# zssjh/stereo-semantic-vo

Hardware: AMD Instinct MI355X
Metric: stereo frames/sec on KITTI 00 (full Tracking::Track chain) (higher is better)
Workload: dtype u8; 1 GPU; BASELINE configs[2]: synth-kitti00 sequence of 4541 distinct 1241x376 stereo pairs, full Tracking::Track loop per frame (ORB on L and R, sparse stereo, matching passes 1+2, PnP-RANSAC, pose-only LM, map-point lifecycle); ONE sequence per GPU in strict frame order (replicas across GPUs); parallelism=one GPU, resident_pairs_per_gpu=4541, resident_input_bytes_per_gpu=4370984960, frames_tracked=4541, tracker_capacity_flag=0, pnp_samples_through_sequential_fallback=0

## Files before the change

### stereo-semantic-vo_amd/csrc/svo_epnp_ord_asm.h

```cpp
#define EO_JACOBI_ASM_12 \
  "v_mov_b64 v[150:151], %[x0]\n\t" \
  "v_mov_b64 v[152:153], %[x1]\n\t" \
  "v_mov_b64 v[154:155], %[x2]\n\t" \
  "v_mov_b64 v[180:181], 1.0\n\t" \
  "v_mov_b32 v254, 1\n\t" \
  "ds_read_b32 v158, %[tper] offset:0\n\t" \
  "ds_read_b32 v159, %[tper] offset:48\n\t" \
  "ds_read_b32 v176, %[tper] offset:96\n\t" \
  "ds_read_b32 v177, %[tper] offset:144\n\t" \
  "ds_read_b32 v178, %[tper] offset:192\n\t" \
  "ds_read_b32 v179, %[tper] offset:240\n\t" \
  "ds_read_b32 v246, %[tper] offset:288\n\t" \
  "ds_read_b32 v247, %[tper] offset:336\n\t" \
  "ds_read_b32 v248, %[tper] offset:384\n\t" \
  "ds_read_b32 v249, %[tper] offset:432\n\t" \
  "ds_read_b32 v250, %[tper] offset:480\n\t" \
  "ds_read_b32 v251, %[tper] offset:528\n\t" \
  "v_and_b32 v228, 15, %[lane]\n\t" \
  "v_sub_u32 v230, v228, %[base]\n\t" \
  "v_cmp_ne_u32 s[60:61], 0, %[act]\n\t" \
  "s_waitcnt lgkmcnt(0)\n\t" \
  "v_and_b32 v253, 15, v158\n\t" \
  "v_cmp_ne_u32 vcc, v253, v230\n\t" \
  "s_and_b64 s[62:63], vcc, s[60:61]\n\t" \
// ... 3659 lines not shown
  "v_and_b32 v246, 0x80, v234\n\t" \
  "v_cmp_ne_u32 vcc, 0, v246\n\t" \
  "s_and_b64 s[68:69], vcc, s[60:61]\n\t" \
  "s_cbranch_scc0 L_open_%=\n\t" \
  "v_bfe_u32 v246, v234, 8, 2\n\t" \
  "v_add_u32 v246, v246, v240\n\t" \
  "v_lshrrev_b32 v247, v246, %[chg]\n\t" \
  "v_and_b32 v247, 1, v247\n\t" \
  "v_cmp_ne_u32 vcc, 0, v247\n\t" \
  "s_and_b64 s[70:71], vcc, s[68:69]\n\t" \
  "v_mov_b32 v247, s70\n\t" \
  "v_and_b32 v247, v247, %[pm]\n\t" \
  "v_cmp_eq_u32 vcc, 0, v247\n\t" \
  "v_cmp_le_u32 s[70:71], 24, v246\n\t" \
  "s_or_b64 vcc, vcc, s[70:71]\n\t" \
  "s_and_b64 vcc, vcc, s[68:69]\n\t" \
  "s_andn2_b64 s[60:61], s[60:61], vcc\n\t" \
  "s_and_b64 s[70:71], s[70:71], s[68:69]\n\t" \
  "v_cndmask_b32_e64 v246, 0, 1, s[70:71]\n\t" \
  "v_or_b32 %[flag], %[flag], v246\n\t" \
  "s_and_b64 s[62:63], s[62:63], s[60:61]\n\t" \
  "L_open_%=:\n\t" \
  "v_mov_b32 v234, v235\n\t" \
  "v_mov_b32 v240, v241\n\t" \
  "v_mov_b32 v241, v239\n\t" \
  "s_cmp_lg_u64 s[60:61], 0\n\t" \
  "s_cbranch_scc1 L_loop_%=\n\t" \
  "L_done_%=:\n\t" \
  "s_waitcnt lgkmcnt(0)\n\t" \
  "v_mov_b64 %[x0], v[150:151]\n\t" \
  "v_mov_b64 %[x1], v[152:153]\n\t" \
  "v_mov_b64 %[x2], v[154:155]\n\t"

#define EO_JACOBI_ASM_CLOBBERS "v140", "v141", "v142", "v143", "v144", "v145", "v146", "v147", "v148", "v149", "v150", "v151", "v152", "v153", "v154", "v155", "v156", "v157", "v158", "v159", "v160", "v161", "v162", "v163", "v164", "v165", "v166", "v167", "v168", "v169", "v170", "v171", "v172", "v173", "v174", "v175", "v176", "v177", "v178", "v179", "v180", "v181", "v182", "v183", "v184", "v185", "v186", "v187", "v188", "v189", "v190", "v191", "v192", "v193", "v194", "v195", "v196", "v197", "v198", "v199", "v200", "v201", "v202", "v203", "v204", "v205", "v206", "v207", "v208", "v209", "v210", "v211", "v212", "v213", "v214", "v215", "v216", "v217", "v218", "v219", "v220", "v221", "v222", "v223", "v224", "v225", "v226", "v227", "v228", "v229", "v230", "v231", "v232", "v233", "v234", "v235", "v236", "v237", "v238", "v239", "v240", "v241", "v242", "v243", "v244", "v245", "v246", "v247", "v248", "v249", "v250", "v251", "v252", "v253", "v254", "v255", "s60", "s61", "s62", "s63", "s64", "s65", "s66", "s67", "s68", "s69", "s70", "s71", "vcc", "scc", "memory"
```

### stereo-semantic-vo_amd/csrc/svo_epnp_ord_dev.h

```cpp
#pragma once
#ifndef HIP_INCLUDE_HIP_HIP_RUNTIME_H
#include <hip/hip_runtime.h>
#endif
#include <stdint.h>

#include "svo_epnp_exact_dev.h"

namespace epnp_ord {

#define EO_FN __device__ __forceinline__
typedef double d2 __attribute__((ext_vector_type(2)));

#include "svo_epnp_ord_tab.h"
#include "svo_epnp_ord_asm.h"

#define EO_SYNC()                                         \
  do {                                                    \
    __builtin_amdgcn_fence(__ATOMIC_ACQ_REL, "wavefront"); \
    __builtin_amdgcn_wave_barrier();                      \
  } while (0)

struct Lds {
  alignas(16) double jr[16 * 16];
  alignas(16) double xch[16][4][4];
  unsigned tab[EO_TAB_TOTAL];
  double pws[16], us[10], alphas[20], cws[12], ccinv[9];
  double M[120];
  double ut4[4][12];
  double L[60], rho[6];
  double sw[3][6];
  double bx[3][6];
  double ccs[3][12], pcs[3][16], abt[3][9], Rc[3][9], rep[3][8];
  alignas(16) double gn[3][6][6];
  double out[3][16];
  int srow[3][6];
  int urow[4];
  double xw[16];
  int flag;
  int sweeps;
  int why;
  long long stamp[8];
#ifdef EO_PROFILE
  long long prof[8];
#endif
};

EO_FN double xdiv(double a, double b) { return a / b; }
EO_FN double xsqrt(double x) { return sqrt(x); }

EO_FN double ndiv(double a, double b) {
  double r = __builtin_amdgcn_rcp(b);
  double e = __builtin_fma(-b, r, 1.0);
  r = __builtin_fma(r, e, r);
  e = __builtin_fma(-b, r, 1.0);
  r = __builtin_fma(r, e, r);
  const double q = a * r;
  const double rem = __builtin_fma(-b, q, a);
  return __builtin_fma(rem, r, q);
}
EO_FN double nsqrt(double x) {
  const double y = __builtin_amdgcn_rsq(x);
  double g = x * y, h = 0.5 * y;
  const double r = __builtin_fma(-h, g, 0.5);
  g = __builtin_fma(g, r, g);
  h = __builtin_fma(h, r, h);
  double d = __builtin_fma(-g, g, x);
  g = __builtin_fma(d, h, g);
  d = __builtin_fma(-g, g, x);
  g = __builtin_fma(d, h, g);
  return g;
}
EO_FN bool w_in_range(double w) { return w >= 7.888609052210118e-31 && w <= 1.2676506002282294e30; }

EO_FN double gsum(double term, double acc) { return __builtin_amdgcn_mfma_f64_4x4x4f64(1.0, term, acc, 0, 0, 0); }
template <int M>
EO_FN double colsum(double t0, double t1, double t2, int g) {
// ... 104 lines not shown
        "v_mul_f64 %[s2], %[n2], %[n2]\n\t"
        "v_mfma_f64_4x4x4_4b_f64 %[a], %[one], %[s0], 0\n\t"
        "s_nop 3\n\t"
        "v_mfma_f64_4x4x4_4b_f64 %[a], %[one], %[s1], %[a]\n\t"
        "s_nop 3\n\t"
        "v_mfma_f64_4x4x4_4b_f64 %[a], %[one], %[s2], %[a]\n\t"
        "s_nop 5"
        : [a] "=&v"(a), [s0] "=&v"(s0), [s1] "=&v"(s1), [s2] "=&v"(s2)
        : [n0] "v"(n0), [n1] "v"(n1), [n2] "v"(n2), [one] "v"(one));
  } else if (M == 6) {
    asm volatile(
        "v_mul_f64 %[s0], %[n0], %[n0]\n\t"
        "v_mul_f64 %[s1], %[n1], %[n1]\n\t"
        "v_mul_f64 %[s1], %[s1], %[mk]\n\t"
        "v_mfma_f64_4x4x4_4b_f64 %[a], %[one], %[s0], 0\n\t"
        "s_nop 3\n\t"
        "v_mfma_f64_4x4x4_4b_f64 %[a], %[one], %[s1], %[a]\n\t"
        "s_nop 5"
        : [a] "=&v"(a), [s0] "=&v"(s0), [s1] "=&v"(s1)
        : [n0] "v"(n0), [n1] "v"(n1), [mk] "v"(mk), [one] "v"(one));
  } else {
    asm volatile(
        "v_mul_f64 %[s0], %[n0], %[n0]\n\t"
        "v_mul_f64 %[s0], %[s0], %[mk]\n\t"
        "s_nop 1\n\t"
        "v_mfma_f64_4x4x4_4b_f64 %[a], %[one], %[s0], 0\n\t"
        "s_nop 5"
        : [a] "=&v"(a), [s0] "=&v"(s0)
        : [n0] "v"(n0), [mk] "v"(mk), [one] "v"(one));
  }
  return a;
}

template <int M>
EO_FN unsigned long long jacobi_rows(Lds& S, int n, int base, int lane) {
  const int r = lane & 15, g = lane >> 4, q = r - base;
  const double mk = M == 6 ? (g < 2 ? 1.0 : 0.0) : (M == 3 ? (g < 3 ? 1.0 : 0.0) : 1.0);
  const double eps = 2.220446049250313e-16 * 10;
  double x0 = S.jr[r * 16 + g], x1 = S.jr[r * 16 + 4 + g], x2 = S.jr[r * 16 + 8 + g];
  double* const mine = S.xch[r][g];
  { d2 lo; lo.x = x0; lo.y = x1; *reinterpret_cast<d2*>(mine) = lo; mine[2] = x2; }
  const int tb = n == 12 ? EO_TAB12_OFF : (n == 5 ? EO_TAB5_OFF : (n == 4 ? EO_TAB4_OFF : EO_TAB3_OFF));
  const int steps = n == 12 ? EO_TAB12_STEPS : (n == 5 ? EO_TAB5_STEPS : (n == 4 ? EO_TAB4_STEPS : EO_TAB3_STEPS));
  const int pro = n == 12 ? EO_TAB12_PROLOGUE : (n == 5 ? EO_TAB5_PROLOGUE : (n == 4 ? EO_TAB4_PROLOGUE : EO_TAB3_PROLOGUE));
  static_assert(EO_TAB3_SWEEPS == 1 && EO_TAB4_SWEEPS == 1 && EO_TAB5_SWEEPS == 1 && EO_TAB12_SWEEPS == 1, "one sweep per period");
  auto lds = [](const void* p) { return (unsigned)(unsigned long long)p; };
  const unsigned a_tab = lds(&S.tab[0]);
  const unsigned twrap = a_tab + 4u * (unsigned)(n > 0 ? tb + pro * n + q : 0);
  const unsigned cfg = (unsigned)steps | (unsigned)pro << 8 | (unsigned)(4 * n) << 16;
  const unsigned pm = n > 0 ? ((1u << n) - 1u) << base : 0u;
  EO_SYNC();
  const double eps2 = eps * eps;
  const double eps2hi = eps2 * (1.0 + 9.094947017729282e-13), eps2lo = eps2 * (1.0 - 9.094947017729282e-13);
  unsigned chg = 0, nst = 0, flag = 0;
  int tt = 0, tp = n > 0 ? tb + q : 0, sb = 0;
  const unsigned e0 = S.tab[tp];
  ++tt; tp += n;
  if (tt == steps) { tt = pro; tp = n > 0 ? tb + pro * n + q : 0; ++sb; }
  const unsigned e1 = S.tab[tp];
  const unsigned tpa = a_tab + 4u * (unsigned)tp;
  const unsigned act = n >= 2 ? 1u : 0u;
  const unsigned amine = lds(mine), axch = lds(&S.xch[0][g][0]);
#define EO_JACOBI_OPERANDS                                                                                                       \
  : [x0] "+v"(x0), [x1] "+v"(x1), [x2] "+v"(x2), [chg] "+v"(chg), [nst] "+v"(nst), [flag] "+v"(flag)                              \
  : [e0] "v"(e0), [e1] "v"(e1), [tt] "v"(tt), [tp] "v"(tpa), [sb] "v"(sb), [cfg] "v"(cfg), [twrap] "v"(twrap), [lane] "v"(lane), \
    [base] "v"(base), [act] "v"(act), [pm] "v"(pm), [mk] "v"(mk), [eps] "v"(eps), [eps2hi] "v"(eps2hi), [eps2lo] "v"(eps2lo),   \
    [amine] "v"(amine), [axch] "v"(axch)                                                                                          \
  : EO_JACOBI_ASM_CLOBBERS
  if (M == 12)
    asm volatile(EO_JACOBI_ASM_12
                 : [x0] "+v"(x0), [x1] "+v"(x1), [x2] "+v"(x2), [chg] "+v"(chg), [flag] "+v"(flag)
                 : [tper] "v"(twrap), [lane] "v"(lane), [base] "v"(base), [act] "v"(act), [pm] "v"(pm), [eps] "v"(eps),
                   [eps2hi] "v"(eps2hi), [eps2lo] "v"(eps2lo), [amine] "v"(amine), [axch] "v"(axch)
                 : EO_JACOBI_ASM_CLOBBERS);
  else if (M == 6) asm volatile(EO_JACOBI_ASM_6 EO_JACOBI_OPERANDS);
  else asm volatile(EO_JACOBI_ASM_3 EO_JACOBI_OPERANDS);
#undef EO_JACOBI_OPERANDS
  const unsigned long long exhausted = __ballot(flag != 0 && n > 0);
  if (M == 12 && flag) S.why |= 1;
  if (M == 12 && lane == 0) S.sweeps = (int)nst;
  const double w = xsqrt(row_norm2<M>(x0, x1, x2, mk));
  const double sc1 = 1 / w;
  if (n > 0) {
    S.jr[r * 16 + g] = M >= 4 || g < M ? x0 * sc1 : x0;
    S.jr[r * 16 + 4 + g] = M >= 8 || 4 + g < M ? x1 * sc1 : x1;
    S.jr[r * 16 + 8 + g] = M >= 12 || 8 + g < M ? x2 * sc1 : x2;
    if (g == 0) S.jr[r * 16 + 15] = w;
  }
  EO_SYNC();
  return exhausted;
}

EO_FN unsigned long long svd_rank(Lds& S, int n, int base, int p, int lane) {
  const int col = lane & 15;
  bool bad = false;
  if (col < n) {
    const double my = S.jr[(base + col) * 16 + 15];
    int rank = 0;
    bad = !w_in_range(my);
    for (int q = 0; q < 5; ++q)
      if (q < n && q != col) {
        const double o = S.jr[(base + q) * 16 + 15];
        rank += o > my ? 1 : 0;
        bad = bad || o == my;
      }
    S.sw[p][rank] = my;
    S.srow[p][rank] = base + col;
  }
  EO_SYNC();
  return __ballot(bad);
// ... 209 lines not shown
  }
}

EO_FN double dot3(const double* a, const double* b) { return a[0] * b[0] + a[1] * b[1] + a[2] * b[2]; }

EO_FN bool solve5_wave(Lds& S, epnp_exact::Work& xw, const double* K, double* R_out, double* t_out, double* rep, bool force_seq = false) {
  const int lane = threadIdx.x & 63, slot = lane >> 4, col = lane & 15, r16 = lane & 15;
  const double fu = K[0], fv = K[1], uc = K[2], vc = K[3];
  if (lane == 0) { S.flag = force_seq ? 1 : 0; S.why = force_seq ? 16 : 0; S.stamp[0] = clock64(); }
  load_tables(S, lane);
  EO_SYNC();
  if (lane < 3) {
    double c = 0;
    for (int i = 0; i < 5; i++) c += S.pws[3 * i + lane];
    S.cws[lane] = c / 5;
  }
  EO_SYNC();
  auto load_pw0 = [&]() {
    if (lane < 9) {
      const int a = lane / 3, b = lane % 3;
      const double ca = S.cws[a], cb = S.cws[b];
      double s = 0;
      for (int i = 0; i < 5; ++i) s += (S.pws[3 * i + a] - ca) * (S.pws[3 * i + b] - cb);
      S.jr[b * 16 + a] = s;
    } else if (lane < 18) {
      const int r = (lane - 9) / 3, k = (lane - 9) % 3;
      S.jr[r * 16 + 3 + k] = r == k ? 1.0 : 0.0;
    } else if (lane < 36) {
      S.jr[((lane - 18) / 6) * 16 + 6 + (lane - 18) % 6] = 0.0;
    }
    EO_SYNC();
  };
  load_pw0();
  unsigned long long ex = jacobi_rows<3>(S, r16 < 3 ? 3 : 0, r16 < 3 ? 0 : r16, lane);
  unsigned long long bd = svd_rank(S, slot == 0 ? 3 : 0, 0, 0, lane);
  if (ex | bd) {
    load_pw0();
    if (lane == 0) svd_small_seq(S, xw.jW, 3, 3, 0, 0);
    EO_SYNC();
  }
  if (lane < 9) {
    const int i = 1 + lane / 3, j = lane % 3;
    const double k = xsqrt(S.sw[0][i - 1] / 5);
    S.cws[3 * i + j] = S.cws[j] + k * S.jr[S.srow[0][i - 1] * 16 + j];
  }
  EO_SYNC();
  auto load_cc = [&]() {
    if (lane < 9) {
      const int r = lane / 3, k = lane % 3;
      S.jr[r * 16 + k] = S.cws[3 * (r + 1) + k] - S.cws[k];
    } else if (lane < 18) {
      const int r = (lane - 9) / 3, k = (lane - 9) % 3;
      S.jr[r * 16 + 3 + k] = r == k ? 1.0 : 0.0;
    } else if (lane < 36) {
      S.jr[((lane - 18) / 6) * 16 + 6 + (lane - 18) % 6] = 0.0;
    }
    EO_SYNC();
  };
  load_cc();
  ex = jacobi_rows<3>(S, r16 < 3 ? 3 : 0, r16 < 3 ? 0 : r16, lane);
  bd = svd_rank(S, slot == 0 ? 3 : 0, 0, 0, lane);
  if (ex | bd) {
    load_cc();
    if (lane == 0) svd_small_seq(S, xw.jW, 3, 3, 0, 0);
    EO_SYNC();
  }
  if (lane < 9) {
    const int j = lane / 3, c = lane % 3;
    double threshold = 0;
    for (int i = 0; i < 3; ++i) threshold += S.sw[0][i];
    threshold *= 2.220446049250313e-16 * 2;
    double x = 0;
    for (int i = 0; i < 3; ++i) {
      double wi = S.sw[0][i];
      if (fabs(wi) <= threshold) continue;
      wi = 1 / wi;
      const int r = S.srow[0][i];
      double s = S.jr[r * 16 + c];
      s *= wi;
      x = x + s * S.jr[r * 16 + 3 + j];
    }
    S.ccinv[lane] = x;
  }
  EO_SYNC();
  if (lane < 15) {
    const int i = lane / 3, j = lane % 3;
    const double* ci = S.ccinv;
    const double* pi = S.pws + 3 * i;
    S.alphas[4 * i + 1 + j] = ci[3 * j] * (pi[0] - S.cws[0]) + ci[3 * j + 1] * (pi[1] - S.cws[1]) + ci[3 * j + 2] * (pi[2] - S.cws[2]);
  }
  EO_SYNC();
  if (lane < 5) {
    const double* a = S.alphas + 4 * lane;
// ... 135 lines not shown
    const int i = col / 3, j = col % 3;
    const double* a = S.alphas + 4 * i;
    const double* cc = S.ccs[cand];
    S.pcs[cand][col] = a[0] * cc[j] + a[1] * cc[3 + j] + a[2] * cc[6 + j] + a[3] * cc[9 + j];
  }
  EO_SYNC();
  double pc0[3], pw0[3];
  bool flip;
  {
    const double* pc = S.pcs[cand];
    flip = pc[2] < 0.0;
    for (int j = 0; j < 3; ++j) { pc0[j] = 0; pw0[j] = 0; }
    for (int i = 0; i < 5; ++i)
      for (int j = 0; j < 3; ++j) { pc0[j] += flip ? -pc[3 * i + j] : pc[3 * i + j]; pw0[j] += S.pws[3 * i + j]; }
    for (int j = 0; j < 3; ++j) { pc0[j] /= 5; pw0[j] /= 5; }
  }
  auto load_abt = [&](int only) {
    const double* pc = S.pcs[cand];
    if (slot < 3 && (only < 0 || slot == only) && col < 9) {
      const int j = col / 3, k = col % 3;
      double s = 0;
      for (int i = 0; i < 5; ++i) s += ((flip ? -pc[3 * i + j] : pc[3 * i + j]) - pc0[j]) * (S.pws[3 * i + k] - pw0[k]);
      S.jr[(base + k) * 16 + j] = s;
    } else if (slot < 3 && (only < 0 || slot == only) && col < 12) {
      const int r = col - 9;
      for (int k = 0; k < 3; ++k) S.jr[(base + r) * 16 + 3 + k] = r == k ? 1.0 : 0.0;
      for (int k = 6; k < 12; ++k) S.jr[(base + r) * 16 + k] = 0.0;
    }
    EO_SYNC();
  };
  load_abt(-1);
  {
    const bool mine = r16 < 15 && r16 % 5 < 3;
    ex = jacobi_rows<3>(S, mine ? 3 : 0, mine ? 5 * (r16 / 5) : r16, lane);
  }
  bd = svd_rank(S, slot < 3 ? 3 : 0, base, cand, lane);
  if (ex | bd) {
    const unsigned need = need_seq(ex, bd);
    for (int pp = 0; pp < 3; ++pp)
      if (need >> pp & 1) load_abt(pp);
    if (slot < 3 && col == 0 && (need >> slot & 1)) svd_small_seq(S, slot == 0 ? xw.jW : (slot == 1 ? xw.sA : xw.sUt), 3, 3, base, cand);
    EO_SYNC();
  }
  if (slot < 3 && col < 9) {
    const int i = col / 3, j = col % 3;
    const int r0 = S.srow[cand][0], r1 = S.srow[cand][1], r2 = S.srow[cand][2];
    S.Rc[cand][col] = S.jr[r0 * 16 + i] * S.jr[r0 * 16 + 3 + j] + S.jr[r1 * 16 + i] * S.jr[r1 * 16 + 3 + j] + S.jr[r2 * 16 + i] * S.jr[r2 * 16 + 3 + j];
  }
  EO_SYNC();
  double R[9], t[3];
  for (int k = 0; k < 9; ++k) R[k] = S.Rc[cand][k];
  {
    const double det = R[0] * R[4] * R[8] + R[1] * R[5] * R[6] + R[2] * R[3] * R[7] - R[2] * R[4] * R[6] - R[1] * R[3] * R[8] - R[0] * R[5] * R[7];
    if (det < 0) { R[6] = -R[6]; R[7] = -R[7]; R[8] = -R[8]; }
  }
  t[0] = pc0[0] - dot3(R, pw0); t[1] = pc0[1] - dot3(R + 3, pw0); t[2] = pc0[2] - dot3(R + 6, pw0);
  if (slot < 3 && col < 5) {
    const double* pw = S.pws + 3 * col;
    const double Xc = dot3(R, pw) + t[0], Yc = dot3(R + 3, pw) + t[1], inv_Zc = 1.0 / (dot3(R + 6, pw) + t[2]);
    const double ue = uc + fu * Xc * inv_Zc, ve = vc + fv * Yc * inv_Zc;
    const double u = S.us[2 * col], v = S.us[2 * col + 1];
    S.rep[cand][col] = xsqrt((u - ue) * (u - ue) + (v - ve) * (v - ve));
  }
  EO_SYNC();
  if (slot < 3 && col == 0) {
    double sum2 = 0.0;
    for (int i = 0; i < 5; ++i) sum2 += S.rep[cand][i];
// ... 40 lines not shown
```

Baseline: 9972 stereo frames/s.

## Run 3x3 one-sided Jacobi sweeps entirely in registers without LDS exchange

For the M==3 Jacobi SVD used in EPnP, each lane now loads all three rows of its 3-column problem into registers. It performs the three fixed (0,1),(0,2),(1,2) rotations per sweep inline, with no LDS exchange buffer or rotation-table lookups. Sweep termination uses a scalar counter capped at 25. The point is to remove LDS round-trips and table-driven pairing from the small 3x3 SVDs. In exchange each lane carries redundant register state and the assembly is hand-written, with a compile-time flag to fall back to the table path. Profiling hooks are added only under EO_PROFILE.

```diff
diff --git a/stereo-semantic-vo_amd/csrc/svo_epnp_ord_asm.h b/stereo-semantic-vo_amd/csrc/svo_epnp_ord_asm.h
--- a/stereo-semantic-vo_amd/csrc/svo_epnp_ord_asm.h
+++ b/stereo-semantic-vo_amd/csrc/svo_epnp_ord_asm.h
@@ -3715,4 +3715,434 @@
   "v_mov_b64 %[x1], v[152:153]\n\t" \
   "v_mov_b64 %[x2], v[154:155]\n\t"
 
+#define EO_JACOBI_ASM_3R \
+  "v_mov_b64 v[180:181], 1.0\n\t" \
+  "ds_read2_b64 v[234:237], %[ajr] offset0:0 offset1:4\n\t" \
+  "ds_read2_b64 v[238:241], %[ajr] offset0:16 offset1:20\n\t" \
+  "ds_read2_b64 v[242:245], %[ajr] offset0:32 offset1:36\n\t" \
+  "v_and_b32 v246, 15, %[lane]\n\t" \
+  "v_sub_u32 v246, v246, %[base]\n\t" \
+  "v_cmp_ne_u32 s[60:61], 0, %[act]\n\t" \
+  "s_mov_b64 s[68:69], 0\n\t" \
+  "s_mov_b32 s66, 0\n\t" \
+  "s_waitcnt lgkmcnt(0)\n\t" \
+  "s_cmp_lg_u64 s[60:61], 0\n\t" \
+  "s_cbranch_scc0 L_done_%=\n\t" \
+  ".p2align 6\n\t" \
+  "L_loop_%=:\n\t" \
+  "v_mul_f64 v[140:141], v[234:235], v[234:235]\n\t" \
+  "v_mul_f64 v[182:183], v[234:235], v[238:239]\n\t" \
+  "v_mul_f64 v[146:147], v[238:239], v[238:239]\n\t" \
+  "v_mul_f64 v[182:183], v[182:183], %[mk]\n\t" \
+  "v_mul_f64 v[140:141], v[140:141], %[mk]\n\t" \
+  "v_mul_f64 v[146:147], v[146:147], %[mk]\n\t" \
+  "s_nop 0\n\t" \
+  "v_mfma_f64_4x4x4_4b_f64 v[156:157], v[180:181], v[140:141], 0\n\t" \
+  "v_mfma_f64_4x4x4_4b_f64 v[210:211], v[180:181], v[146:147], 0\n\t" \
+  "v_mfma_f64_4x4x4_4b_f64 v[200:201], v[180:181], v[182:183], 0\n\t" \
+  "s_nop 4\n\t" \
+  "v_mul_f64 v[188:189], v[156:157], v[210:211]\n\t" \
+  "v_mul_f64 v[192:193], v[200:201], v[200:201]\n\t" \
+  "v_mul_f64 v[194:195], v[188:189], %[eps2hi]\n\t" \
+  "v_mul_f64 v[196:197], v[188:189], %[eps2lo]\n\t" \
+  "v_cmp_gt_f64 vcc, v[192:193], v[194:195]\n\t" \
+  "v_cmp_lt_f64 s[70:71], v[192:193], v[196:197]\n\t" \
+  "s_or_b64 s[70:71], vcc, s[70:71]\n\t" \
+  "s_andn2_b64 s[70:71], s[60:61], s[70:71]\n\t" \
+  "s_cbranch_scc0 L_decided_0_%=\n\t" \
+  "v_rsq_f64 v[190:191], v[188:189]\n\t" \
+  "s_nop 0\n\t" \
+  "v_mul_f64 v[202:203], v[188:189], v[190:191]\n\t" \
+  "v_mul_f64 v[194:195], v[190:191], 0.5\n\t" \
+  "v_fma_f64 v[196:197], -v[194:195], v[202:203], 0.5\n\t" \
+  "v_fma_f64 v[202:203], v[202:203], v[196:197], v[202:203]\n\t" \
+  "v_fma_f64 v[194:195], v[194:195], v[196:197], v[194:195]\n\t" \
+  "v_fma_f64 v[198:199], -v[202:203], v[202:203], v[188:189]\n\t" \
+  "v_fma_f64 v[202:203], v[198:199], v[194:195], v[202:203]\n\t" \
+  "v_fma_f64 v[198:199], -v[202:203], v[202:203], v[188:189]\n\t" \
+  "v_fma_f64 v[202:203], v[198:199], v[194:195], v[202:203]\n\t" \
+  "v_mul_f64 v[202:203], v[202:203], %[eps]\n\t" \
+  "v_cmp_nle_f64 vcc, |v[200:201]|, v[202:203]\n\t" \
+  "L_decided_0_%=:\n\t" \
+  "s_and_b64 s[64:65], vcc, s[60:61]\n\t" \
+  "s_cbranch_scc0 L_skip_0_%=\n\t" \
+  "v_add_f64 v[200:201], v[200:201], v[200:201]\n\t" \
+  "v_add_f64 v[212:213], v[156:157], -v[210:211]\n\t" \
+  "v_cmp_gt_f64 vcc, |v[200:201]|, |v[212:213]|\n\t" \
+  "s_nop 1\n\t" \
+  "v_cndmask_b32 v214, v212, v200, vcc\n\t" \
+  "v_cndmask_b32 v215, v213, v201, vcc\n\t" \
+  "v_cndmask_b32 v216, v200, v212, vcc\n\t" \
+  "v_cndmask_b32 v217, v201, v213, vcc\n\t" \
+  "v_rcp_f64 v[160:161], |v[214:215]|\n\t" \
+  "s_nop 0\n\t" \
+  "v_fma_f64 v[162:163], -|v[214:215]|, v[160:161], 1.0\n\t" \
+  "v_fma_f64 v[160:161], v[160:161], v[162:163], v[160:161]\n\t" \
+  "v_fma_f64 v[162:163], -|v[214:215]|, v[160:161], 1.0\n\t" \
+  "v_fma_f64 v[160:161], v[160:161], v[162:163], v[160:161]\n\t" \
+  "v_mul_f64 v[166:167], |v[216:217]|, v[160:161]\n\t" \
+  "v_fma_f64 v[164:165], -|v[214:215]|, v[166:167], |v[216:217]|\n\t" \
+  "v_fma_f64 v[166:167], v[164:165], v[160:161], v[166:167]\n\t" \
+  "v_mul_f64 v[168:169], v[166:167], v[166:167]\n\t" \
+  "v_add_f64 v[168:169], v[168:169], 1.0\n\t" \
+  "v_rsq_f64 v[190:191], v[168:169]\n\t" \
+  "s_nop 0\n\t" \
+  "v_mul_f64 v[170:171], v[168:169], v[190:191]\n\t" \
+  "v_mul_f64 v[194:195], v[190:191], 0.5\n\t" \
+  "v_fma_f64 v[196:197], -v[194:195], v[170:171], 0.5\n\t" \
+  "v_fma_f64 v[170:171], v[170:171], v[196:197], v[170:171]\n\t" \
+  "v_fma_f64 v[194:195], v[194:195], v[196:197], v[194:195]\n\t" \
+  "v_fma_f64 v[198:199], -v[170:171], v[170:171], v[168:169]\n\t" \
+  "v_fma_f64 v[170:171], v[198:199], v[194:195], v[170:171]\n\t" \
+  "v_fma_f64 v[198:199], -v[170:171], v[170:171], v[168:169]\n\t" \
+  "v_fma_f64 v[170:171], v[198:199], v[194:195], v[170:171]\n\t" \
+  "v_mul_f64 v[218:219], |v[214:215]|, v[170:171]\n\t" \
+  "v_add_f64 v[168:169], v[218:219], |v[212:213]|\n\t" \
+  "v_add_f64 v[172:173], v[218:219], v[218:219]\n\t" \
+  "v_rcp_f64 v[160:161], v[172:173]\n\t" \
+  "s_nop 0\n\t" \
+  "v_fma_f64 v[162:163], -v[172:173], v[160:161], 1.0\n\t" \
+  "v_fma_f64 v[160:161], v[160:161], v[162:163], v[160:161]\n\t" \
+  "v_fma_f64 v[162:163], -v[172:173], v[160:161], 1.0\n\t" \
+  "v_fma_f64 v[160:161], v[160:161], v[162:163], v[160:161]\n\t" \
+  "v_mul_f64 v[166:167], v[168:169], v[160:161]\n\t" \
+  "v_fma_f64 v[164:165], -v[172:173], v[166:167], v[168:169]\n\t" \
+  "v_fma_f64 v[166:167], v[164:165], v[160:161], v[166:167]\n\t" \
+  "v_rsq_f64 v[190:191], v[166:167]\n\t" \
+  "s_nop 0\n\t" \
+  "v_mul_f64 v[220:221], v[166:167], v[190:191]\n\t" \
+  "v_mul_f64 v[194:195], v[190:191], 0.5\n\t" \
+  "v_fma_f64 v[196:197], -v[194:195], v[220:221], 0.5\n\t" \
+  "v_fma_f64 v[220:221], v[220:221], v[196:197], v[220:221]\n\t" \
+  "v_fma_f64 v[194:195], v[194:195], v[196:197], v[194:195]\n\t" \
+  "v_fma_f64 v[198:199], -v[220:221], v[220:221], v[166:167]\n\t" \
+  "v_fma_f64 v[220:221], v[198:199], v[194:195], v[220:221]\n\t" \
+  "v_fma_f64 v[198:199], -v[220:221], v[220:221], v[166:167]\n\t" \
+  "v_fma_f64 v[220:221], v[198:199], v[194:195], v[220:221]\n\t" \
+  "v_mul_f64 v[168:169], v[218:219], v[220:221]\n\t" \
+  "v_add_f64 v[168:169], v[168:169], v[168:169]\n\t" \
+  "v_rcp_f64 v[160:161], v[168:169]\n\t" \
+  "s_nop 0\n\t" \
+  "v_fma_f64 v[162:163], -v[168:169], v[160:161], 1.0\n\t" \
+  "v_fma_f64 v[160:161], v[160:161], v[162:163], v[160:161]\n\t" \
+  "v_fma_f64 v[162:163], -v[168:169], v[160:161], 1.0\n\t" \
+  "v_fma_f64 v[160:161], v[160:161], v[162:163], v[160:161]\n\t" \
+  "v_mul_f64 v[222:223], v[200:201], v[160:161]\n\t" \
+  "v_fma_f64 v[164:165], -v[168:169], v[222:223], v[200:201]\n\t" \
+  "v_fma_f64 v[222:223], v[164:165], v[160:161], v[222:223]\n\t" \
+  "v_cmp_gt_f64 vcc, 0, v[212:213]\n\t" \
+  "s_nop 1\n\t" \
+  "v_cndmask_b32 v226, v222, v220, vcc\n\t" \
+  "v_cndmask_b32 v227, v223, v221, vcc\n\t" \
+  "v_cndmask_b32 v224, v220, v222, vcc\n\t" \
+  "v_cndmask_b32 v225, v221, v223, vcc\n\t" \
+  "v_mul_f64 v[228:229], v[224:225], v[234:235]\n\t" \
+  "v_mul_f64 v[182:183], v[226:227], v[238:239]\n\t" \
+  "v_mul_f64 v[230:231], v[224:225], v[236:237]\n\t" \
+  "v_mul_f64 v[184:185], v[226:227], v[240:241]\n\t" \
+  "v_mul_f64 v[186:187], -v[226:227], v[234:235]\n\t" \
+  "v_mul_f64 v[232:233], v[224:225], v[238:239]\n\t" \
+  "v_mul_f64 v[140:141], -v[226:227], v[236:237]\n\t" \
+  "v_mul_f64 v[146:147], v[224:225], v[240:241]\n\t" \
+  "v_add_f64 v[228:229], v[228:229], v[182:183]\n\t" \
+  "v_add_f64 v[230:231], v[230:231], v[184:185]\n\t" \
+  "v_add_f64 v[232:233], v[186:187], v[232:233]\n\t" \
+  "v_add_f64 v[146:147], v[140:141], v[146:147]\n\t" \
+  "v_cndmask_b32_e64 v234, v234, v228, s[64:65]\n\t" \
+  "v_cndmask_b32_e64 v235, v235, v229, s[64:65]\n\t" \
+  "v_cndmask_b32_e64 v236, v236, v230, s[64:65]\n\t" \
+  "v_cndmask_b32_e64 v237, v237, v231, s[64:65]\n\t" \
+  "v_cndmask_b32_e64 v238, v238, v232, s[64:65]\n\t" \
+  "v_cndmask_b32_e64 v239, v239, v233, s[64:65]\n\t" \
+  "v_cndmask_b32_e64 v240, v240, v146, s[64:65]\n\t" \
+  "v_cndmask_b32_e64 v241, v241, v147, s[64:65]\n\t" \
+  "s_or_b64 s[68:69], s[68:69], s[64:65]\n\t" \
+  "L_skip_0_%=:\n\t" \
+  "v_mul_f64 v[140:141], v[234:235], v[234:235]\n\t" \
+  "v_mul_f64 v[182:183], v[234:235], v[242:243]\n\t" \
+  "v_mul_f64 v[146:147], v[242:243], v[242:243]\n\t" \
+  "v_mul_f64 v[182:183], v[182:183], %[mk]\n\t" \
+  "v_mul_f64 v[140:141], v[140:141], %[mk]\n\t" \
+  "v_mul_f64 v[146:147], v[146:147], %[mk]\n\t" \
+  "s_nop 0\n\t" \
+  "v_mfma_f64_4x4x4_4b_f64 v[156:157], v[180:181], v[140:141], 0\n\t" \
+  "v_mfma_f64_4x4x4_4b_f64 v[210:211], v[180:181], v[146:147], 0\n\t" \
+  "v_mfma_f64_4x4x4_4b_f64 v[200:201], v[180:181], v[182:183], 0\n\t" \
+  "s_nop 4\n\t" \
+  "v_mul_f64 v[188:189], v[156:157], v[210:211]\n\t" \
+  "v_mul_f64 v[192:193], v[200:201], v[200:201]\n\t" \
+  "v_mul_f64 v[194:195], v[188:189], %[eps2hi]\n\t" \
+  "v_mul_f64 v[196:197], v[188:189], %[eps2lo]\n\t" \
+  "v_cmp_gt_f64 vcc, v[192:193], v[194:195]\n\t" \
+  "v_cmp_lt_f64 s[70:71], v[192:193], v[196:197]\n\t" \
+  "s_or_b64 s[70:71], vcc, s[70:71]\n\t" \
+  "s_andn2_b64 s[70:71], s[60:61], s[70:71]\n\t" \
+  "s_cbranch_scc0 L_decided_1_%=\n\t" \
+  "v_rsq_f64 v[190:191], v[188:189]\n\t" \
+  "s_nop 0\n\t" \
+  "v_mul_f64 v[202:203], v[188:189], v[190:191]\n\t" \
+  "v_mul_f64 v[194:195], v[190:191], 0.5\n\t" \
+  "v_fma_f64 v[196:197], -v[194:195], v[202:203], 0.5\n\t" \
+  "v_fma_f64 v[202:203], v[202:203], v[196:197], v[202:203]\n\t" \
+  "v_fma_f64 v[194:195], v[194:195], v[196:197], v[194:195]\n\t" \
+  "v_fma_f64 v[198:199], -v[202:203], v[202:203], v[188:189]\n\t" \
+  "v_fma_f64 v[202:203], v[198:199], v[194:195], v[202:203]\n\t" \
+  "v_fma_f64 v[198:199], -v[202:203], v[202:203], v[188:189]\n\t" \
+  "v_fma_f64 v[202:203], v[198:199], v[194:195], v[202:203]\n\t" \
+  "v_mul_f64 v[202:203], v[202:203], %[eps]\n\t" \
+  "v_cmp_nle_f64 vcc, |v[200:201]|, v[202:203]\n\t" \
+  "L_decided_1_%=:\n\t" \
+  "s_and_b64 s[64:65], vcc, s[60:61]\n\t" \
+  "s_cbranch_scc0 L_skip_1_%=\n\t" \
+  "v_add_f64 v[200:201], v[200:201], v[200:201]\n\t" \
+  "v_add_f64 v[212:213], v[156:157], -v[210:211]\n\t" \
+  "v_cmp_gt_f64 vcc, |v[200:201]|, |v[212:213]|\n\t" \
+  "s_nop 1\n\t" \
+  "v_cndmask_b32 v214, v212, v200, vcc\n\t" \
+  "v_cndmask_b32 v215, v213, v201, vcc\n\t" \
+  "v_cndmask_b32 v216, v200, v212, vcc\n\t" \
+  "v_cndmask_b32 v217, v201, v213, vcc\n\t" \
+  "v_rcp_f64 v[160:161], |v[214:215]|\n\t" \
+  "s_nop 0\n\t" \
+  "v_fma_f64 v[162:163], -|v[214:215]|, v[160:161], 1.0\n\t" \
+  "v_fma_f64 v[160:161], v[160:161], v[162:163], v[160:161]\n\t" \
+  "v_fma_f64 v[162:163], -|v[214:215]|, v[160:161], 1.0\n\t" \
+  "v_fma_f64 v[160:161], v[160:161], v[162:163], v[160:161]\n\t" \
+  "v_mul_f64 v[166:167], |v[216:217]|, v[160:161]\n\t" \
+  "v_fma_f64 v[164:165], -|v[214:215]|, v[166:167], |v[216:217]|\n\t" \
+  "v_fma_f64 v[166:167], v[164:165], v[160:161], v[166:167]\n\t" \
+  "v_mul_f64 v[168:169], v[166:167], v[166:167]\n\t" \
+  "v_add_f64 v[168:169], v[168:169], 1.0\n\t" \
+  "v_rsq_f64 v[190:191], v[168:169]\n\t" \
+  "s_nop 0\n\t" \
+  "v_mul_f64 v[170:171], v[168:169], v[190:191]\n\t" \
+  "v_mul_f64 v[194:195], v[190:191], 0.5\n\t" \
+  "v_fma_f64 v[196:197], -v[194:195], v[170:171], 0.5\n\t" \
+  "v_fma_f64 v[170:171], v[170:171], v[196:197], v[170:171]\n\t" \
+  "v_fma_f64 v[194:195], v[194:195], v[196:197], v[194:195]\n\t" \
+  "v_fma_f64 v[198:199], -v[170:171], v[170:171], v[168:169]\n\t" \
+  "v_fma_f64 v[170:171], v[198:199], v[194:195], v[170:171]\n\t" \
+  "v_fma_f64 v[198:199], -v[170:171], v[170:171], v[168:169]\n\t" \
+  "v_fma_f64 v[170:171], v[198:199], v[194:195], v[170:171]\n\t" \
+  "v_mul_f64 v[218:219], |v[214:215]|, v[170:171]\n\t" \
+  "v_add_f64 v[168:169], v[218:219], |v[212:213]|\n\t" \
+  "v_add_f64 v[172:173], v[218:219], v[218:219]\n\t" \
+  "v_rcp_f64 v[160:161], v[172:173]\n\t" \
+  "s_nop 0\n\t" \
+  "v_fma_f64 v[162:163], -v[172:173], v[160:161], 1.0\n\t" \
+  "v_fma_f64 v[160:161], v[160:161], v[162:163], v[160:161]\n\t" \
+  "v_fma_f64 v[162:163], -v[172:173], v[160:161], 1.0\n\t" \
+  "v_fma_f64 v[160:161], v[160:161], v[162:163], v[160:161]\n\t" \
+  "v_mul_f64 v[166:167], v[168:169], v[160:161]\n\t" \
+  "v_fma_f64 v[164:165], -v[172:173], v[166:167], v[168:169]\n\t" \
+  "v_fma_f64 v[166:167], v[164:165], v[160:161], v[166:167]\n\t" \
+  "v_rsq_f64 v[190:191], v[166:167]\n\t" \
+  "s_nop 0\n\t" \
+  "v_mul_f64 v[220:221], v[166:167], v[190:191]\n\t" \
+  "v_mul_f64 v[194:195], v[190:191], 0.5\n\t" \
+  "v_fma_f64 v[196:197], -v[194:195], v[220:221], 0.5\n\t" \
+  "v_fma_f64 v[220:221], v[220:221], v[196:197], v[220:221]\n\t" \
+  "v_fma_f64 v[194:195], v[194:195], v[196:197], v[194:195]\n\t" \
+  "v_fma_f64 v[198:199], -v[220:221], v[220:221], v[166:167]\n\t" \
+  "v_fma_f64 v[220:221], v[198:199], v[194:195], v[220:221]\n\t" \
+  "v_fma_f64 v[198:199], -v[220:221], v[220:221], v[166:167]\n\t" \
+  "v_fma_f64 v[220:221], v[198:199], v[194:195], v[220:221]\n\t" \
+  "v_mul_f64 v[168:169], v[218:219], v[220:221]\n\t" \
+  "v_add_f64 v[168:169], v[168:169], v[168:169]\n\t" \
+  "v_rcp_f64 v[160:161], v[168:169]\n\t" \
+  "s_nop 0\n\t" \
+  "v_fma_f64 v[162:163], -v[168:169], v[160:161], 1.0\n\t" \
+  "v_fma_f64 v[160:161], v[160:161], v[162:163], v[160:161]\n\t" \
+  "v_fma_f64 v[162:163], -v[168:169], v[160:161], 1.0\n\t" \
+  "v_fma_f64 v[160:161], v[160:161], v[162:163], v[160:161]\n\t" \
+  "v_mul_f64 v[222:223], v[200:201], v[160:161]\n\t" \
+  "v_fma_f64 v[164:165], -v[168:169], v[222:223], v[200:201]\n\t" \
+  "v_fma_f64 v[222:223], v[164:165], v[160:161], v[222:223]\n\t" \
+  "v_cmp_gt_f64 vcc, 0, v[212:213]\n\t" \
+  "s_nop 1\n\t" \
+  "v_cndmask_b32 v226, v222, v220, vcc\n\t" \
+  "v_cndmask_b32 v227, v223, v221, vcc\n\t" \
+  "v_cndmask_b32 v224, v220, v222, vcc\n\t" \
+  "v_cndmask_b32 v225, v221, v223, vcc\n\t" \
+  "v_mul_f64 v[228:229], v[224:225], v[234:235]\n\t" \
+  "v_mul_f64 v[182:183], v[226:227], v[242:243]\n\t" \
+  "v_mul_f64 v[230:231], v[224:225], v[236:237]\n\t" \
+  "v_mul_f64 v[184:185], v[226:227], v[244:245]\n\t" \
+  "v_mul_f64 v[186:187], -v[226:227], v[234:235]\n\t" \
+  "v_mul_f64 v[232:233], v[224:225], v[242:243]\n\t" \
+  "v_mul_f64 v[140:141], -v[226:227], v[236:237]\n\t" \
+  "v_mul_f64 v[146:147], v[224:225], v[244:245]\n\t" \
+  "v_add_f64 v[228:229], v[228:229], v[182:183]\n\t" \
+  "v_add_f64 v[230:231], v[230:231], v[184:185]\n\t" \
+  "v_add_f64 v[232:233], v[186:187], v[232:233]\n\t" \
+  "v_add_f64 v[146:147], v[140:141], v[146:147]\n\t" \
+  "v_cndmask_b32_e64 v234, v234, v228, s[64:65]\n\t" \
+  "v_cndmask_b32_e64 v235, v235, v229, s[64:65]\n\t" \
+  "v_cndmask_b32_e64 v236, v236, v230, s[64:65]\n\t" \
+  "v_cndmask_b32_e64 v237, v237, v231, s[64:65]\n\t" \
+  "v_cndmask_b32_e64 v242, v242, v232, s[64:65]\n\t" \
+  "v_cndmask_b32_e64 v243, v243, v233, s[64:65]\n\t" \
+  "v_cndmask_b32_e64 v244, v244, v146, s[64:65]\n\t" \
+  "v_cndmask_b32_e64 v245, v245, v147, s[64:65]\n\t" \
+  "s_or_b64 s[68:69], s[68:69], s[64:65]\n\t" \
+  "L_skip_1_%=:\n\t" \
+  "v_mul_f64 v[140:141], v[238:239], v[238:239]\n\t" \
+  "v_mul_f64 v[182:183], v[238:239], v[242:243]\n\t" \
+  "v_mul_f64 v[146:147], v[242:243], v[242:243]\n\t" \
+  "v_mul_f64 v[182:183], v[182:183], %[mk]\n\t" \
+  "v_mul_f64 v[140:141], v[140:141], %[mk]\n\t" \
+  "v_mul_f64 v[146:147], v[146:147], %[mk]\n\t" \
+  "s_nop 0\n\t" \
+  "v_mfma_f64_4x4x4_4b_f64 v[156:157], v[180:181], v[140:141], 0\n\t" \
+  "v_mfma_f64_4x4x4_4b_f64 v[210:211], v[180:181], v[146:147], 0\n\t" \
+  "v_mfma_f64_4x4x4_4b_f64 v[200:201], v[180:181], v[182:183], 0\n\t" \
+  "s_nop 4\n\t" \
+  "v_mul_f64 v[188:189], v[156:157], v[210:211]\n\t" \
+  "v_mul_f64 v[192:193], v[200:201], v[200:201]\n\t" \
+  "v_mul_f64 v[194:195], v[188:189], %[eps2hi]\n\t" \
+  "v_mul_f64 v[196:197], v[188:189], %[eps2lo]\n\t" \
+  "v_cmp_gt_f64 vcc, v[192:193], v[194:195]\n\t" \
+  "v_cmp_lt_f64 s[70:71], v[192:193], v[196:197]\n\t" \
+  "s_or_b64 s[70:71], vcc, s[70:71]\n\t" \
+  "s_andn2_b64 s[70:71], s[60:61], s[70:71]\n\t" \
+  "s_cbranch_scc0 L_decided_2_%=\n\t" \
+  "v_rsq_f64 v[190:191], v[188:189]\n\t" \
+  "s_nop 0\n\t" \
+  "v_mul_f64 v[202:203], v[188:189], v[190:191]\n\t" \
+  "v_mul_f64 v[194:195], v[190:191], 0.5\n\t" \
+  "v_fma_f64 v[196:197], -v[194:195], v[202:203], 0.5\n\t" \
+  "v_fma_f64 v[202:203], v[202:203], v[196:197], v[202:203]\n\t" \
+  "v_fma_f64 v[194:195], v[194:195], v[196:197], v[194:195]\n\t" \
+  "v_fma_f64 v[198:199], -v[202:203], v[202:203], v[188:189]\n\t" \
+  "v_fma_f64 v[202:203], v[198:199], v[194:195], v[202:203]\n\t" \
+  "v_fma_f64 v[198:199], -v[202:203], v[202:203], v[188:189]\n\t" \
+  "v_fma_f64 v[202:203], v[198:199], v[194:195], v[202:203]\n\t" \
+  "v_mul_f64 v[202:203], v[202:203], %[eps]\n\t" \
+  "v_cmp_nle_f64 vcc, |v[200:201]|, v[202:203]\n\t" \
+  "L_decided_2_%=:\n\t" \
+  "s_and_b64 s[64:65], vcc, s[60:61]\n\t" \
+  "s_cbranch_scc0 L_skip_2_%=\n\t" \
+  "v_add_f64 v[200:201], v[200:201], v[200:201]\n\t" \
+  "v_add_f64 v[212:213], v[156:157], -v[210:211]\n\t" \
+  "v_cmp_gt_f64 vcc, |v[200:201]|, |v[212:213]|\n\t" \
+  "s_nop 1\n\t" \
+  "v_cndmask_b32 v214, v212, v200, vcc\n\t" \
+  "v_cndmask_b32 v215, v213, v201, vcc\n\t" \
+  "v_cndmask_b32 v216, v200, v212, vcc\n\t" \
+  "v_cndmask_b32 v217, v201, v213, vcc\n\t" \
+  "v_rcp_f64 v[160:161], |v[214:215]|\n\t" \
+  "s_nop 0\n\t" \
+  "v_fma_f64 v[162:163], -|v[214:215]|, v[160:161], 1.0\n\t" \
+  "v_fma_f64 v[160:161], v[160:161], v[162:163], v[160:161]\n\t" \
+  "v_fma_f64 v[162:163], -|v[214:215]|, v[160:161], 1.0\n\t" \
+  "v_fma_f64 v[160:161], v[160:161], v[162:163], v[160:161]\n\t" \
+  "v_mul_f64 v[166:167], |v[216:217]|, v[160:161]\n\t" \
+  "v_fma_f64 v[164:165], -|v[214:215]|, v[166:167], |v[216:217]|\n\t" \
+  "v_fma_f64 v[166:167], v[164:165], v[160:161], v[166:167]\n\t" \
+  "v_mul_f64 v[168:169], v[166:167], v[166:167]\n\t" \
+  "v_add_f64 v[168:169], v[168:169], 1.0\n\t" \
+  "v_rsq_f64 v[190:191], v[168:169]\n\t" \
+  "s_nop 0\n\t" \
+  "v_mul_f64 v[170:171], v[168:169], v[190:191]\n\t" \
+  "v_mul_f64 v[194:195], v[190:191], 0.5\n\t" \
+  "v_fma_f64 v[196:197], -v[194:195], v[170:171], 0.5\n\t" \
+  "v_fma_f64 v[170:171], v[170:171], v[196:197], v[170:171]\n\t" \
+  "v_fma_f64 v[194:195], v[194:195], v[196:197], v[194:195]\n\t" \
+  "v_fma_f64 v[198:199], -v[170:171], v[170:171], v[168:169]\n\t" \
+  "v_fma_f64 v[170:171], v[198:199], v[194:195], v[170:171]\n\t" \
+  "v_fma_f64 v[198:199], -v[170:171], v[170:171], v[168:169]\n\t" \
+  "v_fma_f64 v[170:171], v[198:199], v[194:195], v[170:171]\n\t" \
+  "v_mul_f64 v[218:219], |v[214:215]|, v[170:171]\n\t" \
+  "v_add_f64 v[168:169], v[218:219], |v[212:213]|\n\t" \
+  "v_add_f64 v[172:173], v[218:219], v[218:219]\n\t" \
+  "v_rcp_f64 v[160:161], v[172:173]\n\t" \
+  "s_nop 0\n\t" \
+  "v_fma_f64 v[162:163], -v[172:173], v[160:161], 1.0\n\t" \
+  "v_fma_f64 v[160:161], v[160:161], v[162:163], v[160:161]\n\t" \
+  "v_fma_f64 v[162:163], -v[172:173], v[160:161], 1.0\n\t" \
+  "v_fma_f64 v[160:161], v[160:161], v[162:163], v[160:161]\n\t" \
+  "v_mul_f64 v[166:167], v[168:169], v[160:161]\n\t" \
+  "v_fma_f64 v[164:165], -v[172:173], v[166:167], v[168:169]\n\t" \
+  "v_fma_f64 v[166:167], v[164:165], v[160:161], v[166:167]\n\t" \
+  "v_rsq_f64 v[190:191], v[166:167]\n\t" \
+  "s_nop 0\n\t" \
+  "v_mul_f64 v[220:221], v[166:167], v[190:191]\n\t" \
+  "v_mul_f64 v[194:195], v[190:191], 0.5\n\t" \
+  "v_fma_f64 v[196:197], -v[194:195], v[220:221], 0.5\n\t" \
+  "v_fma_f64 v[220:221], v[220:221], v[196:197], v[220:221]\n\t" \
+  "v_fma_f64 v[194:195], v[194:195], v[196:197], v[194:195]\n\t" \
+  "v_fma_f64 v[198:199], -v[220:221], v[220:221], v[166:167]\n\t" \
+  "v_fma_f64 v[220:221], v[198:199], v[194:195], v[220:221]\n\t" \
+  "v_fma_f64 v[198:199], -v[220:221], v[220:221], v[166:167]\n\t" \
+  "v_fma_f64 v[220:221], v[198:199], v[194:195], v[220:221]\n\t" \
+  "v_mul_f64 v[168:169], v[218:219], v[220:221]\n\t" \
+  "v_add_f64 v[168:169], v[168:169], v[168:169]\n\t" \
+  "v_rcp_f64 v[160:161], v[168:169]\n\t" \
+  "s_nop 0\n\t" \
+  "v_fma_f64 v[162:163], -v[168:169], v[160:161], 1.0\n\t" \
+  "v_fma_f64 v[160:161], v[160:161], v[162:163], v[160:161]\n\t" \
+  "v_fma_f64 v[162:163], -v[168:169], v[160:161], 1.0\n\t" \
+  "v_fma_f64 v[160:161], v[160:161], v[162:163], v[160:161]\n\t" \
+  "v_mul_f64 v[222:223], v[200:201], v[160:161]\n\t" \
+  "v_fma_f64 v[164:165], -v[168:169], v[222:223], v[200:201]\n\t" \
+  "v_fma_f64 v[222:223], v[164:165], v[160:161], v[222:223]\n\t" \
+  "v_cmp_gt_f64 vcc, 0, v[212:213]\n\t" \
+  "s_nop 1\n\t" \
+  "v_cndmask_b32 v226, v222, v220, vcc\n\t" \
+  "v_cndmask_b32 v227, v223, v221, vcc\n\t" \
+  "v_cndmask_b32 v224, v220, v222, vcc\n\t" \
+  "v_cndmask_b32 v225, v221, v223, vcc\n\t" \
+  "v_mul_f64 v[228:229], v[224:225], v[238:239]\n\t" \
+  "v_mul_f64 v[182:183], v[226:227], v[242:243]\n\t" \
+  "v_mul_f64 v[230:231], v[224:225], v[240:241]\n\t" \
+  "v_mul_f64 v[184:185], v[226:227], v[244:245]\n\t" \
+  "v_mul_f64 v[186:187], -v[226:227], v[238:239]\n\t" \
+  "v_mul_f64 v[232:233], v[224:225], v[242:243]\n\t" \
+  "v_mul_f64 v[140:141], -v[226:227], v[240:241]\n\t" \
+  "v_mul_f64 v[146:147], v[224:225], v[244:245]\n\t" \
+  "v_add_f64 v[228:229], v[228:229], v[182:183]\n\t" \
+  "v_add_f64 v[230:231], v[230:231], v[184:185]\n\t" \
+  "v_add_f64 v[232:233], v[186:187], v[232:233]\n\t" \
+  "v_add_f64 v[146:147], v[140:141], v[146:147]\n\t" \
+  "v_cndmask_b32_e64 v238, v238, v228, s[64:65]\n\t" \
+  "v_cndmask_b32_e64 v239, v239, v229, s[64:65]\n\t" \
+  "v_cndmask_b32_e64 v240, v240, v230, s[64:65]\n\t" \
+  "v_cndmask_b32_e64 v241, v241, v231, s[64:65]\n\t" \
+  "v_cndmask_b32_e64 v242, v242, v232, s[64:65]\n\t" \
+  "v_cndmask_b32_e64 v243, v243, v233, s[64:65]\n\t" \
+  "v_cndmask_b32_e64 v244, v244, v146, s[64:65]\n\t" \
+  "v_cndmask_b32_e64 v245, v245, v147, s[64:65]\n\t" \
+  "s_or_b64 s[68:69], s[68:69], s[64:65]\n\t" \
+  "L_skip_2_%=:\n\t" \
+  "s_mov_b64 s[70:71], s[60:61]\n\t" \
+  "s_and_b64 s[60:61], s[60:61], s[68:69]\n\t" \
+  "s_mov_b64 s[68:69], 0\n\t" \
+  "s_add_u32 s66, s66, 1\n\t" \
+  "s_cmp_lt_u32 s66, 25\n\t" \
+  "s_cbranch_scc1 L_more_%=\n\t" \
+  "v_cndmask_b32_e64 v247, 0, 1, s[70:71]\n\t" \
+  "v_or_b32 %[flag], %[flag], v247\n\t" \
+  "s_mov_b64 s[60:61], 0\n\t" \
+  "L_more_%=:\n\t" \
+  "s_cmp_lg_u64 s[60:61], 0\n\t" \
+  "s_cbranch_scc1 L_loop_%=\n\t" \
+  "L_done_%=:\n\t" \
+  "v_mov_b64 v[150:151], v[234:235]\n\t" \
+  "v_mov_b64 v[152:153], v[236:237]\n\t" \
+  "v_cmp_eq_u32 vcc, 1, v246\n\t" \
+  "s_nop 1\n\t" \
+  "v_cndmask_b32 v150, v150, v238, vcc\n\t" \
+  "v_cndmask_b32 v151, v151, v239, vcc\n\t" \
+  "v_cndmask_b32 v152, v152, v240, vcc\n\t" \
+  "v_cndmask_b32 v153, v153, v241, vcc\n\t" \
+  "v_cmp_eq_u32 vcc, 2, v246\n\t" \
+  "s_nop 1\n\t" \
+  "v_cndmask_b32 v150, v150, v242, vcc\n\t" \
+  "v_cndmask_b32 v151, v151, v243, vcc\n\t" \
+  "v_cndmask_b32 v152, v152, v244, vcc\n\t" \
+  "v_cndmask_b32 v153, v153, v245, vcc\n\t" \
+  "v_mov_b32 %[chg], s66\n\t" \
+  "v_mov_b64 %[x0], v[150:151]\n\t" \
+  "v_mov_b64 %[x1], v[152:153]\n\t"
+
 #define EO_JACOBI_ASM_CLOBBERS "v140", "v141", "v142", "v143", "v144", "v145", "v146", "v147", "v148", "v149", "v150", "v151", "v152", "v153", "v154", "v155", "v156", "v157", "v158", "v159", "v160", "v161", "v162", "v163", "v164", "v165", "v166", "v167", "v168", "v169", "v170", "v171", "v172", "v173", "v174", "v175", "v176", "v177", "v178", "v179", "v180", "v181", "v182", "v183", "v184", "v185", "v186", "v187", "v188", "v189", "v190", "v191", "v192", "v193", "v194", "v195", "v196", "v197", "v198", "v199", "v200", "v201", "v202", "v203", "v204", "v205", "v206", "v207", "v208", "v209", "v210", "v211", "v212", "v213", "v214", "v215", "v216", "v217", "v218", "v219", "v220", "v221", "v222", "v223", "v224", "v225", "v226", "v227", "v228", "v229", "v230", "v231", "v232", "v233", "v234", "v235", "v236", "v237", "v238", "v239", "v240", "v241", "v242", "v243", "v244", "v245", "v246", "v247", "v248", "v249", "v250", "v251", "v252", "v253", "v254", "v255", "s60", "s61", "s62", "s63", "s64", "s65", "s66", "s67", "s68", "s69", "s70", "s71", "vcc", "scc", "memory"
diff --git a/stereo-semantic-vo_amd/csrc/svo_epnp_ord_dev.h b/stereo-semantic-vo_amd/csrc/svo_epnp_ord_dev.h
--- a/stereo-semantic-vo_amd/csrc/svo_epnp_ord_dev.h
+++ b/stereo-semantic-vo_amd/csrc/svo_epnp_ord_dev.h
@@ -42,6 +42,7 @@
   long long stamp[8];
 #ifdef EO_PROFILE
   long long prof[8];
+  int j3sweeps;
 #endif
 };
 
@@ -212,14 +213,30 @@
   return a;
 }
 
+#ifdef EO_PROFILE
+#define EO_PROF3_BEGIN() if (lane == 0) { S.j3sweeps = 0; S.prof[6] = clock64(); } EO_SYNC()
+#define EO_PROF3_END(idx) if (lane == 0) { S.prof[idx] = clock64() - S.prof[6]; S.prof[3 + (idx)] = S.j3sweeps; } EO_SYNC()
+#else
+#define EO_PROF3_BEGIN() do {} while (0)
+#define EO_PROF3_END(idx) do {} while (0)
+#endif
+
 template <int M>
 EO_FN unsigned long long jacobi_rows(Lds& S, int n, int base, int lane) {
   const int r = lane & 15, g = lane >> 4, q = r - base;
   const double mk = M == 6 ? (g < 2 ? 1.0 : 0.0) : (M == 3 ? (g < 3 ? 1.0 : 0.0) : 1.0);
   const double eps = 2.220446049250313e-16 * 10;
-  double x0 = S.jr[r * 16 + g], x1 = S.jr[r * 16 + 4 + g], x2 = S.jr[r * 16 + 8 + g];
+#ifdef EO_JACOBI3_TABLE
+  constexpr bool regs3 = false;
+#else
+  constexpr bool regs3 = M == 3;
+#endif
+  double x0 = 0, x1 = 0, x2 = S.jr[r * 16 + 8 + g];
   double* const mine = S.xch[r][g];
-  { d2 lo; lo.x = x0; lo.y = x1; *reinterpret_cast<d2*>(mine) = lo; mine[2] = x2; }
+  if (!regs3) {
+    x0 = S.jr[r * 16 + g]; x1 = S.jr[r * 16 + 4 + g];
+    d2 lo; lo.x = x0; lo.y = x1; *reinterpret_cast<d2*>(mine) = lo; mine[2] = x2;
+  }
   const int tb = n == 12 ? EO_TAB12_OFF : (n == 5 ? EO_TAB5_OFF : (n == 4 ? EO_TAB4_OFF : EO_TAB3_OFF));
   const int steps = n == 12 ? EO_TAB12_STEPS : (n == 5 ? EO_TAB5_STEPS : (n == 4 ? EO_TAB4_STEPS : EO_TAB3_STEPS));
   const int pro = n == 12 ? EO_TAB12_PROLOGUE : (n == 5 ? EO_TAB5_PROLOGUE : (n == 4 ? EO_TAB4_PROLOGUE : EO_TAB3_PROLOGUE));
@@ -234,10 +251,10 @@
   const double eps2hi = eps2 * (1.0 + 9.094947017729282e-13), eps2lo = eps2 * (1.0 - 9.094947017729282e-13);
   unsigned chg = 0, nst = 0, flag = 0;
   int tt = 0, tp = n > 0 ? tb + q : 0, sb = 0;
-  const unsigned e0 = S.tab[tp];
+  const unsigned e0 = regs3 ? 0u : S.tab[tp];
   ++tt; tp += n;
   if (tt == steps) { tt = pro; tp = n > 0 ? tb + pro * n + q : 0; ++sb; }
-  const unsigned e1 = S.tab[tp];
+  const unsigned e1 = regs3 ? 0u : S.tab[tp];
   const unsigned tpa = a_tab + 4u * (unsigned)tp;
   const unsigned act = n >= 2 ? 1u : 0u;
   const unsigned amine = lds(mine), axch = lds(&S.xch[0][g][0]);
@@ -254,8 +271,22 @@
                    [eps2hi] "v"(eps2hi), [eps2lo] "v"(eps2lo), [amine] "v"(amine), [axch] "v"(axch)
                  : EO_JACOBI_ASM_CLOBBERS);
   else if (M == 6) asm volatile(EO_JACOBI_ASM_6 EO_JACOBI_OPERANDS);
-  else asm volatile(EO_JACOBI_ASM_3 EO_JACOBI_OPERANDS);
+  else if (!regs3) asm volatile(EO_JACOBI_ASM_3 EO_JACOBI_OPERANDS);
+  else {
+    const unsigned ajr = lds(&S.jr[(n > 0 ? base : 0) * 16 + g]);
+    asm volatile(EO_JACOBI_ASM_3R
+                 : [x0] "=&v"(x0), [x1] "=&v"(x1), [chg] "=&v"(chg), [flag] "+v"(flag)
+                 : [ajr] "v"(ajr), [lane] "v"(lane), [base] "v"(base), [act] "v"(act), [mk] "v"(mk), [eps] "v"(eps), [eps2hi] "v"(eps2hi),
+                   [eps2lo] "v"(eps2lo)
+                 : EO_JACOBI_ASM_CLOBBERS);
+  }
 #undef EO_JACOBI_OPERANDS
+#ifdef EO_PROFILE
+  if (M == 3) {
+    const int sw = regs3 ? (int)chg : (33 - __clz(chg) < 25 ? 33 - __clz(chg) : 25);
+    if (n > 0) atomicMax(&S.j3sweeps, sw);
+  }
+#endif
   const unsigned long long exhausted = __ballot(flag != 0 && n > 0);
   if (M == 12 && flag) S.why |= 1;
   if (M == 12 && lane == 0) S.sweeps = (int)nst;
@@ -531,7 +562,9 @@
     EO_SYNC();
   };
   load_pw0();
+  EO_PROF3_BEGIN();
   unsigned long long ex = jacobi_rows<3>(S, r16 < 3 ? 3 : 0, r16 < 3 ? 0 : r16, lane);
+  EO_PROF3_END(0);
   unsigned long long bd = svd_rank(S, slot == 0 ? 3 : 0, 0, 0, lane);
   if (ex | bd) {
     load_pw0();
@@ -557,7 +590,9 @@
     EO_SYNC();
   };
   load_cc();
+  EO_PROF3_BEGIN();
   ex = jacobi_rows<3>(S, r16 < 3 ? 3 : 0, r16 < 3 ? 0 : r16, lane);
+  EO_PROF3_END(1);
   bd = svd_rank(S, slot == 0 ? 3 : 0, 0, 0, lane);
   if (ex | bd) {
     load_cc();
@@ -759,7 +794,9 @@
   load_abt(-1);
   {
     const bool mine = r16 < 15 && r16 % 5 < 3;
+    EO_PROF3_BEGIN();
     ex = jacobi_rows<3>(S, mine ? 3 : 0, mine ? 5 * (r16 / 5) : r16, lane);
+    EO_PROF3_END(2);
   }
   bd = svd_rank(S, slot < 3 ? 3 : 0, base, cand, lane);
   if (ex | bd) {
```

Measured after the change: 10340 stereo frames/s (median of 6 runs). 1.04x the previous value.
